# WasifurRahman/BERT_multimodal_transformer

Measured on AMD Instinct MI355X. Metric: train samples/sec MAG-BERT MOSI seq_len=50, higher is better.
Workload: dtype bf16; 1 GPU; MAG-BERT bert-base-uncased, MOSI dims (V=47, A=74), batch 48/GPU, seq_len 50, full optimizer step (fwd+MSE+bwd+HF-AdamW+schedule+zero_grad; inputs resident in HBM), dropout on, random-init weights; global_batch=48, seq_len=50, parallelism=dp1, step_call=mb_bert_train_step, hipGraph replay

## Files before the change

### bert_multimodal_transformer_amd/_lib.py

```python
import ctypes as C
import os

_HERE = os.path.dirname(os.path.abspath(__file__))
LIB_PATH = os.path.join(os.environ.get("MB_LIB_DIR") or os.path.join(_HERE, "lib"), "libmagbert_hip.so")

DT_F32, DT_BF16 = 0, 1
GEMM_NT, GEMM_NN, GEMM_TN = 0, 1, 2
EPI_BIAS, EPI_BIAS_GELU, EPI_BIAS_DROP_RES, EPI_ADD_RES, EPI_DGELU, EPI_ACCUM_F32, EPI_BIAS_F32 = range(7)


class DropKey(C.Structure):
    _fields_ = [("k0", C.c_uint32), ("k1", C.c_uint32), ("thresh", C.c_uint32), ("scale", C.c_float)]


class BertEngineConfig(C.Structure):
    _fields_ = [("vocab_size", C.c_int), ("hidden_size", C.c_int), ("num_layers", C.c_int), ("num_heads", C.c_int),
                ("intermediate_size", C.c_int), ("max_position", C.c_int), ("type_vocab", C.c_int),
                ("num_labels", C.c_int), ("visual_dim", C.c_int), ("acoustic_dim", C.c_int), ("pad_token_id", C.c_int),
                ("layer_norm_eps", C.c_float), ("mag_layer_norm_eps", C.c_float), ("beta_shift", C.c_float),
                ("hidden_dropout", C.c_float), ("attn_dropout", C.c_float), ("mag_dropout", C.c_float),
                ("dtype", C.c_int), ("max_batch", C.c_int), ("max_seq", C.c_int)]


class XlnetEngineConfig(C.Structure):
# ... 45 lines not shown
    "mb_bert_sequence_output": (_vp, [_vp]),
    "mb_bert_pooled_output": (_vp, [_vp]),
    "mb_bert_hidden_state": (_vp, [_vp, _i]),
    "mb_bert_set_attention_output": (_i, [_vp, _vp]),
    "mb_debug_gemm_trace": (_i, [_vp, _i]),
    "mb_debug_attention_trace": (_i, [_vp, _i]),
    "mb_xlnet_attention_probs": (_vp, [_vp, _i, C.POINTER(_i)]),
    "mb_xlnet_set_head_mask": (_i, [_vp, _vp]),
    "mb_xlnet_set_perm_mask": (_i, [_vp, _vp]),
    "mb_xlnet_set_mems": (_i, [_vp, _vp, _i]),
    "mb_xlnet_query_stream_scratch_bytes": (_sz, [_vp, _i, _i, _i]),
    "mb_xlnet_query_stream_state_bytes": (_sz, [_vp, _i, _i]),
    "mb_xlnet_query_stream": (_i, [_vp, _vp, _i, _vp, _sz, _vp, _vp]),
    "mb_bert_mark_grads_zero": (_i, [_vp, _i]),
    "mb_xlnet_mark_grads_zero": (_i, [_vp, _i]),
    "mb_bert_materialize_grads": (_i, [_vp, _vp]),
    "mb_xlnet_materialize_grads": (_i, [_vp, _vp]),
    "mb_bert_grads_stale": (_i, [_vp]),
    "mb_xlnet_grads_stale": (_i, [_vp]),
    "mb_bert_set_head_mask": (_i, [_vp, _vp]),
    "mb_bert_set_inputs_embeds": (_i, [_vp, _vp]),
    "mb_bert_set_position_ids": (_i, [_vp, _vp]),
    "mb_bert_inputs_embeds_grad": (_vp, [_vp]),
    "mb_bert_backward_outputs": (_i, [_vp, _vp, _vp, _vp]),
    "mb_bert_stage_grad_ranges": (_i, [_vp, _i, C.POINTER(_sz), C.POINTER(_sz), _i]),
    "mb_bert_train_step": (_i, [_vp, _vp, _vp, _vp, _vp, _vp, _vp, _i, _i, _u64, _u64, _vp, _vp, _vp, _vp, _vp, _f, _f, _f, _f, _f,
                                _i, _i, _f, _f, _i, _vp]),
    "mb_bert_stage_forward": (_i, [_vp, _vp, _vp, _vp, _vp, _vp, _vp, _i, _i, _u64, _u64, _vp, _vp, _vp, _i, _vp]),
    "mb_bert_stage_backward": (_i, [_vp, _f, _i, _i, _vp]),
    "mb_bert_staged_input_ids": (_vp, [_vp]),
# ... 107 lines not shown
```

### bert_multimodal_transformer_amd/bert.py

```python
import ctypes as C
import os

import torch
import torch.nn as nn

from . import _lib
from .global_configs import ACOUSTIC_DIM, VISUAL_DIM


class BertConfig(object):

    def __init__(self, vocab_size=30522, hidden_size=768, num_hidden_layers=12, num_attention_heads=12,
                 intermediate_size=3072, hidden_act="gelu", hidden_dropout_prob=0.1, attention_probs_dropout_prob=0.1,
                 max_position_embeddings=512, type_vocab_size=2, initializer_range=0.02, layer_norm_eps=1e-12,
                 pad_token_id=0, num_labels=1, **kwargs):
        if hidden_act != "gelu":
            raise NotImplementedError("only erf-GELU (bert-base-uncased) is built")
        self.vocab_size = vocab_size
        self.hidden_size = hidden_size
        self.num_hidden_layers = num_hidden_layers
        self.num_attention_heads = num_attention_heads
        self.intermediate_size = intermediate_size
        self.hidden_act = hidden_act
        self.hidden_dropout_prob = hidden_dropout_prob
# ... 393 lines not shown
        self._set_optional(None, None, None)
        ptr, keep = self._inputs(input_ids, visual, acoustic, attention_mask, token_type_ids, labels, gather_in_step=True)
        if not hasattr(self, "_logit_bufs"):
            self._logit_bufs = {}
        logits = self._logit_bufs.get(B)
        if logits is None:
            logits = self._logit_bufs[B] = torch.empty(B, self.config.num_labels, dtype=torch.float32, device=self.device)
        self.step += 1
        self._keep = (keep, logits)
        self._lab_ptr = None
        self.training_last = True
        o = opt or {}
        if comm is not None and opt is None:
            raise ValueError("the data-parallel single-call step ends with the optimizer (micro-steps exchange nothing)")
        extra = () if comm is None else (comm.handle,)
        with _Core._Hop(self):
            _lib.check(self._fn("train_step" if comm is None else "train_step_dp")(
                self.handle, ptr[0], ptr[1], ptr[2], ptr[3], ptr[4], ptr[5], B, L,
                self.seed & (2 ** 64 - 1), self.step, _lib.ptr(logits), C.c_void_p(self.loss_buf.data_ptr()),
                C.c_void_p(self.loss_buf.data_ptr() + 4), _lib.ptr(o.get("m")), _lib.ptr(o.get("v")), o.get("lr", 0.0),
                o.get("beta1", 0.9), o.get("beta2", 0.999), o.get("eps", 1e-6), o.get("weight_decay", 0.0), int(o.get("t", 1)),
                1 if o.get("correct_bias", True) else 0, o.get("grad_scale", 1.0), float(loss_scale), int(mode), self.stream(), *extra))
        self._gz = opt is not None
        self._gz_version = self.grads._version
        return logits

    def stage_step(self, input_ids, visual, acoustic, attention_mask, token_type_ids, labels, loss_scale=1.0, mode=1):
        B, L = input_ids.shape
        self._ensure(B, L)
        if self.weights_dirty:
# ... 514 lines not shown
```

### bert_multimodal_transformer_amd/csrc/adamw.hip

```cpp
#include <cstdlib>
#include "kernels.h"
#include "adamw_dev.h"

namespace mb {

template <bool NT, int UNR, bool CHUNK>
__global__ void __launch_bounds__(256) adamw_var_kernel(float* __restrict__ p, float* __restrict__ g, float* __restrict__ m,
                                                        float* __restrict__ v, bf16* __restrict__ shadow, size_t n4, size_t n_decay,
                                                        size_t sh_begin, size_t sh_end, size_t keep_begin, size_t keep_end, AdamArgs a,
                                                        const AdamArgs* __restrict__ dyn, int zero_grad) {
    if (dyn) a = *dyn;
    const float omb1 = 1.0f - a.beta1, omb2 = 1.0f - a.beta2;
    const float decay = a.lr * a.weight_decay;
    size_t begin, end, stride;
    if constexpr (CHUNK) {
        const size_t per = ((n4 + gridDim.x - 1) / gridDim.x + 255) / 256 * 256;
        begin = (size_t)blockIdx.x * per + threadIdx.x; end = min(n4, (size_t)(blockIdx.x + 1) * per); stride = 256;
    } else {
        begin = (size_t)blockIdx.x * 256 + threadIdx.x; end = n4; stride = (size_t)gridDim.x * 256;
    }
    for (size_t i4 = begin; i4 < end; i4 += stride * UNR) {
        AdamQuad q[UNR];
#pragma unroll
        for (int u = 0; u < UNR; ++u)
// ... 84 lines not shown
        const size_t kb = keep_begin, ke = keep_end;
        const int use = (var == 0 && ke > kb) ? 3 : var;
#define MB_AV(U, C) do { if (nt) hipLaunchKernelGGL((adamw_var_kernel<true, U, C>), dim3(grid), dim3(256), 0, st, p, g, m, v, (bf16*)shadow, n4, n_decay, sh_begin, sh_end, kb, ke, a, dyn, zero_grad); \
                         else hipLaunchKernelGGL((adamw_var_kernel<false, U, C>), dim3(grid), dim3(256), 0, st, p, g, m, v, (bf16*)shadow, n4, n_decay, sh_begin, sh_end, kb, ke, a, dyn, zero_grad); } while (0)
        if (use == 1) MB_AV(2, false); else if (use == 2) MB_AV(1, true); else if (use == 3) MB_AV(2, true); else if (use == 4) MB_AV(4, false); else if (use == 5) MB_AV(4, true); else
#undef MB_AV
        if (nt) hipLaunchKernelGGL(adamw_kernel<true>, dim3(grid), dim3(256), 0, st, p, g, m, v, (bf16*)shadow, n4, n_decay, sh_begin,
                                   sh_end, a, dyn, zero_grad);
        else hipLaunchKernelGGL(adamw_kernel<false>, dim3(grid), dim3(256), 0, st, p, g, m, v, (bf16*)shadow, n4, n_decay, sh_begin,
                                sh_end, a, dyn, zero_grad);
    }
    if (n % 4) hipLaunchKernelGGL(adamw_tail_kernel, dim3(1), dim3(64), 0, st, p, g, m, v, n4 * 4, n, n_decay, a, dyn, zero_grad);
    return (int)hipGetLastError();
}

}
```

### bert_multimodal_transformer_amd/csrc/adamw_dev.h

```cpp
#pragma once
#include "kernels.h"

namespace mb {

struct AdamQuad { f32x4 p, g, m, v; };
template <bool NT> __device__ __forceinline__ AdamQuad adam_load(const float* p, const float* g, const float* m, const float* v, size_t i) {
    AdamQuad q;
    if constexpr (NT) {
        q.p = __builtin_nontemporal_load((const f32x4*)(p + i)); q.g = __builtin_nontemporal_load((const f32x4*)(g + i));
        q.m = __builtin_nontemporal_load((const f32x4*)(m + i)); q.v = __builtin_nontemporal_load((const f32x4*)(v + i));
    } else {
        q.p = *(const f32x4*)(p + i); q.g = *(const f32x4*)(g + i); q.m = *(const f32x4*)(m + i); q.v = *(const f32x4*)(v + i);
    }
    return q;
}
template <bool NT> __device__ __forceinline__ void adam_update_store(AdamQuad q, float* p, float* g, float* m, float* v, bf16* shadow, size_t i,
                                                                     const AdamArgs& a, float omb1, float omb2, float decay, size_t n_decay,
                                                                     size_t sh_begin, size_t sh_end, size_t keep_begin, size_t keep_end, int zero_grad) {
#pragma clang fp contract(off)
    q.g *= a.grad_scale;
    q.m = a.beta1 * q.m + omb1 * q.g;
    q.v = a.beta2 * q.v + omb2 * q.g * q.g;
#pragma unroll
    for (int r = 0; r < 4; ++r) q.p[r] -= a.step_size * (q.m[r] / (sqrtf(q.v[r]) + a.eps));
    if (i < n_decay && decay > 0.f) q.p -= decay * q.p;
    const bool zg = zero_grad && !(i >= keep_begin && i < keep_end);
    if constexpr (NT) {
// ... 49 lines not shown
```

### bert_multimodal_transformer_amd/csrc/engine.hip

```cpp
#include "engine_common.h"
#include "comm.h"

struct LayerOff { size_t wqkv, wo, w1, w2, bqkv, bo, ln1w, ln1b, b1, b2, ln2w, ln2b; };
struct LayerWs { size_t qkv, ctx, s1, st1, y1, u, g, s2, st2, stats; };

struct mb_bert_engine : StepMixin {
    mb_bert_config c;
    std::vector<TensorInfo> tensors;
    std::vector<LayerOff> lo;
    size_t word, pos, type, emb_lnw, emb_lnb, wp, bp, wc, bc;
    size_t mag_whv, mag_wha, mag_wv, mag_wa, mag_bhv, mag_bha, mag_bv, mag_ba, mag_lnw, mag_lnb;
    size_t n_params, n_decay, sh_begin, sh_end;
    MagWs mw;
    size_t ws_mag, ws_emb, ws_emb_st, ws_head_z, ws_head_pooled, ws_logits;
    std::vector<size_t> ws_x;
    std::vector<LayerWs> lw;
    size_t ws_ds[2], ws_dzd[2], ws_ds2[2], ws_dzd2[2], ws_du[2], ws_dqkv[2];
    size_t ws_dxa, ws_dxb, ws_dctx, ws_dsum, ws_dz, ws_lnp_a, ws_lnp_b;
    size_t lnp_stride = 0;
    int lnp_nblk = 0;
    size_t ws_ids, ws_seg, ws_mask, ws_labels;
    size_t ws_bytes;
    float* P = nullptr; float* G = nullptr; char* SH = nullptr; char* ws = nullptr;
    const int64_t* ids = nullptr; const int64_t* seg = nullptr; const int64_t* mask = nullptr;
    int B = 0, L = 0, training = 0;
    int padT = -1;
    hipStream_t side = nullptr;
    std::vector<hipEvent_t> evs;
    int overlap_wgrad = 0;
    int opt_chunk = 0;
    int prefetch = 1;
    int pf_qkv = 0;
    hipStream_t opt_side = nullptr;
    std::vector<hipEvent_t> opt_ev;
    int adam_in_wgrad = 0;
    float* fuse_m = nullptr; float* fuse_v = nullptr;
    int adam_ride = 1, ride_blocks = 0;
    float* ride_m = nullptr; float* ride_v = nullptr;
    size_t ride_cursor = 0;
    long ride_params = 0;
    int ride_dgrad = 2, ride_dgrad_blocks = 0;
    int ride_attn = 1, ride_attn_blocks = 0;
    long ride_attn_params = 0;
    long ride_dgrad_params = 0, ride_dgelu_params = 0;
    int group_wgrad = 256;
    bool grouped = false;
    bool deferred = false;
    float* attn_out = nullptr;
    const float* head_mask = nullptr;
    const float* emb_in = nullptr;
    const int64_t* pos_ids = nullptr;
    bool ran_forward = false;

    bool ws_zeroed = false;
// ... 100 lines not shown
    e->ws_dxa = w.take(T * H * es); e->ws_dxb = w.take(T * H * es);
    for (int k = 0; k < 2; ++k) {
        e->ws_ds[k] = w.take(T * H * es); e->ws_dzd[k] = w.take(T * H * es); e->ws_ds2[k] = w.take(T * H * es);
        e->ws_dzd2[k] = w.take(T * H * es); e->ws_du[k] = w.take(T * I * es); e->ws_dqkv[k] = w.take(T * 3 * H * es);
    }
    e->ws_dctx = w.take(T * H * es); e->ws_dsum = w.take(T * H * 4); e->ws_dz = w.take((size_t)c.max_batch * H * es);
    e->lnp_stride = ln_partials_floats((int)T, (int)H);
    {
        const size_t emb = (size_t)c.max_seq * ((c.max_batch + 7) / 8) * 3 * H;
        if (emb > e->lnp_stride) e->lnp_stride = emb;
    }
    e->ws_lnp_a = w.take(e->lnp_stride * 4 * (c.num_layers + 2)); e->ws_lnp_b = w.take(e->lnp_stride * 4 * (c.num_layers + 2));
    e->carve_step(w, T, (int)V, (int)A, c.max_batch, c.num_labels, SITE_LAYER0 + 4 * c.num_layers);
    e->idcnt_off = w.take((size_t)c.vocab_size * 4);
    { const char* uv = getenv("MB_EMBED_UNIQUE"); e->idcnt_enable = !(uv && atoi(uv) == 0); }
    if (e->deterministic) {
        e->det_begin = e->wp; e->det_end = e->n_params;
        e->ws_det = w.take((e->det_end - e->det_begin) * sizeof(long long));
    }
    e->ws_bytes = w.off;
}

static int ensure_side(mb_bert_engine* e) {
    if (e->side || !e->overlap_wgrad) return MB_OK;
    int least = 0, greatest = 0;
    CK((int)hipDeviceGetStreamPriorityRange(&least, &greatest));
    const char* pv = getenv("MB_SIDE_PRIORITY");
    const int prio = (pv && atoi(pv) != 0) ? least : 0;
    CK((int)hipStreamCreateWithPriority(&e->side, hipStreamNonBlocking, prio));
    e->evs.assign((size_t)e->c.num_layers * 5, nullptr);
// ... 235 lines not shown
    if (ndim) *ndim = t.ndim;
    if (shape4) for (int k = 0; k < 4; ++k) shape4[k] = t.shape[k];
    if (decay) *decay = t.decay;
    return MB_OK;
}
size_t mb_bert_param_count(const mb_bert_engine* e) { return e->n_params; }
size_t mb_bert_decay_count(const mb_bert_engine* e) { return e->n_decay; }
void mb_bert_shadow_range(const mb_bert_engine* e, size_t* b, size_t* en) { *b = e->sh_begin; *en = e->sh_end; }
size_t mb_bert_workspace_bytes(const mb_bert_engine* e) { return e->ws_bytes; }

int mb_bert_bind(mb_bert_engine* e, float* params, float* grads, void* shadow, void* workspace, size_t ws_bytes) {
    if (!params || !workspace || ws_bytes < e->ws_bytes) return MB_ERR_ARG;
    if (e->c.dtype == DT_BF16 && !shadow) return MB_ERR_ARG;
    e->P = params; e->G = grads; e->SH = (char*)shadow; e->ws = (char*)workspace;
    e->grads_zero = false;
    e->ws_zeroed = false; e->padT = -1;
    e->drop_graphs();
    char* mws = e->ws + e->ws_mag;
    e->pkw = {e->P + e->mag_whv, e->P + e->mag_wha, e->P + e->mag_wv, e->P + e->mag_wa, mws + e->mw.We, mws + e->mw.Wv, mws + e->mw.Wa,
              MagDims{0, e->c.hidden_size, e->c.visual_dim, e->c.acoustic_dim, e->mw.Vp, e->mw.Ap}, e->c.dtype};
    return MB_OK;
}

int mb_bert_sync_weights(mb_bert_engine* e, void* stream) {
    hipStream_t st = (hipStream_t)stream;
    if (!e->P) return MB_ERR_ARG;
    if (e->c.dtype == DT_BF16)
        CK(convert(DT_BF16, e->P + e->sh_begin, e->SH + e->sh_begin * 2, e->sh_end - e->sh_begin, st));
    const mb_bert_config& c = e->c;
    MagDims d = {0, c.hidden_size, c.visual_dim, c.acoustic_dim, e->mw.Vp, e->mw.Ap};
// ... 60 lines not shown
    return MB_OK;
}

int mb_bert_forward(mb_bert_engine* e, const int64_t* input_ids, const float* visual, const float* acoustic,
                    const int64_t* attention_mask, const int64_t* token_type_ids, const float* labels, int B, int L,
                    int training, uint64_t seed, uint64_t step, float* logits, float* loss, float* loss_run, void* stream) {
    return bert_forward_range(e, input_ids, visual, acoustic, attention_mask, token_type_ids, labels, B, L, training, seed, step, logits,
                              loss, loss_run, stream, 0, e->c.num_layers, true, true);
}

int mb_bert_backward(mb_bert_engine* e, const float* dlogits, const float* labels, float loss_scale, int stage_begin,
                     int stage_end, void* stream) {
    hipStream_t st = (hipStream_t)stream;
    const mb_bert_config& c = e->c;
    if (!e->G || !e->ran_forward) return MB_ERR_ARG;
    const int dt = c.dtype, H = c.hidden_size, I = c.intermediate_size, B = e->B, L = e->L, T = B * L, nh = c.num_heads;
    const int NL = c.num_layers;
    const int Tk = (int)align_up((size_t)T, 64);
    auto take_ride = [&](int l, size_t budget, int blocks) -> AdamRide {
        AdamRide r = {};
        if (!e->ride_m || !e->ride_v || l + 1 >= e->c.num_layers || blocks < 8 || e->ride_cursor <= e->lo[l + 1].wqkv) return r;
        size_t take = std::min(e->ride_cursor - e->lo[l + 1].wqkv, budget) / 1024 * 1024;
        const size_t re = e->ride_cursor, rb = re - take;
        const bool sh_ok = e->c.dtype != DT_BF16 || (e->sh_begin <= rb && re <= e->sh_end);
        if (take == 0 || rb % 4 || !sh_ok) return r;
        const bool keep = e->keep_in_step() && e->stale_begin <= rb && re <= e->stale_end;
        r = AdamRide{e->P + rb, e->G + rb, e->ride_m + rb, e->ride_v + rb, e->c.dtype == DT_BF16 ? (bf16*)(e->SH + rb * 2) : nullptr,
                     take / 4, e->adam_state(e->ws), blocks / 8 * 8, keep ? 0 : 1};
        e->ride_cursor = rb;
        return r;
// ... 231 lines not shown
    const bool fuse = e->adam_in_wgrad && m && v && nseg == 1 && e->ow_pass && e->grouped && !e->deferred && e->group_wgrad == 128 && NL > 0 &&
                      e->lo[0].wqkv == 0 && !e->prof;
    e->fuse_m = fuse ? m : nullptr; e->fuse_v = fuse ? v : nullptr;
    const bool ride = e->adam_ride && !fuse && m && v && nseg == 1 && e->grouped && !e->deferred && NL > 1 && e->lo[0].wqkv == 0 && !e->prof &&
                      (e->group_wgrad == 128 || e->group_wgrad == 256);
    e->ride_m = ride ? m : nullptr; e->ride_v = ride ? v : nullptr;
    e->ride_cursor = e->wp;
    const int rb = mb_bert_backward(e, nullptr, lab, loss_scale, sb, se, st);
    e->fuse_m = e->fuse_v = nullptr;
    e->ride_m = e->ride_v = nullptr;
    CK(rb);
    if (m && v && seg == nseg - 1) {
        const AdamArgs none = {};
        const size_t nd = e->n_decay, n = e->n_params;
        CK(e->prof_mark(2 * NL, st));
        if (ride) CK(adamw_decay_range(e, m, v, 0, e->ride_cursor, st));
        CK(adamw_decay_range(e, m, v, (nseg == 1 && !fuse && !ride) ? 0 : e->wp, nd, st));
        CK(adamw_step(e->P + nd, e->G + nd, m + nd, v + nd, nullptr, n - nd, 0, 0, 0, none, 1, st, e->adam_state(ws) + 1));
        CK(e->prof_mark(2 * NL + 1, st));
    }
    return MB_OK;
}

static int between_segments(mb_bert_engine* e, int seg, int nseg, float* m, float* v, hipStream_t st) {
    if (nseg == 1 || !m || !v) return MB_OK;
    const int NL = e->c.num_layers, C = NL / (nseg - 1);
    if (seg + 1 < nseg) {
        const int l_lo = NL - (seg + 1) * C, l_hi = NL - seg * C;
        CK((int)hipEventRecord(e->opt_ev[seg], st));
        CK((int)hipStreamWaitEvent(e->opt_side, e->opt_ev[seg], 0));
// ... 234 lines not shown
    return e->prof_span_us(2 * e->c.num_layers, 1, us);
}

const void* mb_bert_hidden_state(const mb_bert_engine* e, int i) {
    if (!e || !e->ws || i < 0 || i > e->c.num_layers) return nullptr;
    return e->ws + e->ws_x[i];
}
int mb_bert_set_attention_output(mb_bert_engine* e, float* probs) {
    if (!e) return MB_ERR_ARG;
    e->attn_out = probs;
    return MB_OK;
}
int mb_bert_mark_grads_zero(mb_bert_engine* e, int known_zero) {
    if (!e) return MB_ERR_ARG;
    e->grads_zero = known_zero != 0;
    if (known_zero) e->grads_stale = false;
    return MB_OK;
}
int mb_bert_materialize_grads(mb_bert_engine* e, void* stream) {
    if (!e) return MB_ERR_ARG;
    return e->materialize_grads(e->G, (hipStream_t)stream);
}
int mb_bert_grads_stale(const mb_bert_engine* e) { return e && e->grads_stale ? 1 : 0; }
int mb_bert_set_head_mask(mb_bert_engine* e, const float* head_mask) {
    if (!e) return MB_ERR_ARG;
    e->head_mask = head_mask;
    return MB_OK;
}
int mb_bert_set_inputs_embeds(mb_bert_engine* e, const float* inputs_embeds) {
    if (!e) return MB_ERR_ARG;
    e->emb_in = inputs_embeds;
    return MB_OK;
}
// ... 62 lines not shown
```

### bert_multimodal_transformer_amd/csrc/engine_common.h

```cpp
#pragma once
#include <string>
#include <vector>
#include <cstring>
#include <cstdio>
#include <cstdlib>
#include <cmath>
#include <algorithm>
#include "kernels.h"
#include "../../include/magbert_hip.h"

using namespace mb;

namespace {

struct TensorInfo {
    std::string name;
    size_t off, numel;
    int ndim;
    int64_t shape[4];
    int decay;
};

inline size_t align_up(size_t x, size_t a) { return (x + a - 1) / a * a; }

// ... 149 lines not shown
        exec.clear(); graph.clear();
    }
};

struct StageGraph { int B, L, stage, overwrite; const void *logits, *loss, *loss_run; float loss_scale; hipStream_t st; hipGraph_t graph; hipGraphExec_t exec; };

struct StepMixin {
    bool dyn = false;
    bool stage_mode = false;
    std::vector<StageGraph> stage_graphs;
    bool pk_enable = false, packed = false;
    bool pkw_enable = false, packed_w = false;
    PrologueArgs::MagPackW pkw = {};
    size_t pk_vis = 0, pk_aco = 0; int pk_Vp = 0, pk_Ap = 0, pk_dtype = 0;
    size_t idcnt_off = 0; bool idcnt_enable = false, counted = false;
    bool loss_cleared = false;
    bool capturing = false;
    int nsites = 0;
    size_t ws_state = 0, ws_in_ids = 0, ws_in_seg = 0, ws_in_mask = 0, ws_in_vis = 0, ws_in_aco = 0, ws_in_lab = 0;
    std::vector<StepGraph> graphs;
    size_t graph_launches = 0, graph_captures = 0;
    hipStream_t cap = nullptr;
    int capture_stream(hipStream_t* out) {
        if (!cap) CK((int)hipStreamCreateWithFlags(&cap, hipStreamNonBlocking));
        *out = cap;
        return MB_OK;
    }
    bool grads_zero = false, ow_pass = false, in_step = false;
    int ow_enable = 1;
    int deterministic = 0;
// ... 11 lines not shown
            if (cus <= 0) cus = 256;
        }
        return cus;
    }
    bool grads_stale = false, ow_covers = false;
    size_t stale_begin = 0, stale_end = 0;
    int keep_enable = 1;
    bool keep_in_step() const { return keep_enable && ow_enable && ow_covers && stale_end > stale_begin; }
    int materialize_grads(float* G, hipStream_t st) {
        if (grads_stale && G) CK(zero_fill(G + stale_begin, (stale_end - stale_begin) * sizeof(float), st));
        grads_stale = false;
        return MB_OK;
    }
    int begin_backward_pass(float* G, hipStream_t st) {
        if (in_step) return MB_OK;
        ow_pass = grads_zero && ow_enable;
        grads_zero = false;
        if (!(ow_pass && ow_covers)) CK(materialize_grads(G, st));
        grads_stale = false;
        return MB_OK;
    }

    bool prof = false;
    std::vector<hipEvent_t> pev;
    int prof_layers = 0;
    int set_profiling(int on, int layers) {
        if (on && pev.empty()) {
            prof_layers = layers;
            pev.assign((size_t)2 * layers + 2, nullptr);
            for (auto& ev : pev) CK((int)hipEventCreate(&ev));
// ... 23 lines not shown
        ws_in_vis = w.take(Tpad * (size_t)V * 4); ws_in_aco = w.take(Tpad * (size_t)A * 4);
        ws_in_lab = w.take((size_t)max_batch * num_labels * 4);
    }
    void drop_graphs() {
        if (cap) { hipStreamDestroy(cap); cap = nullptr; }
        for (auto& g : graphs) g.destroy();
        graphs.clear();
        for (auto& g : stage_graphs) { hipGraphExecDestroy(g.exec); hipGraphDestroy(g.graph); }
        stage_graphs.clear();
    }
    template <class Enq>
    int run_stage_graph(int B, int L, int stage, int overwrite, const void* logits, const void* loss, const void* loss_run, float loss_scale,
                        int mode, hipStream_t st, Enq enqueue) {
        struct Scope { StepMixin* m; ~Scope() { m->dyn = false; m->capturing = false; m->in_step = false; m->stage_mode = false; } } scope{this};
        dyn = true; in_step = true; stage_mode = true;
        if (mode == 2) return enqueue(st);
        StageGraph* g = nullptr;
        for (auto& x : stage_graphs)
            if (x.B == B && x.L == L && x.stage == stage && x.overwrite == overwrite && x.logits == logits && x.loss == loss && x.loss_run == loss_run &&
                x.loss_scale == loss_scale && x.st == st) { g = &x; break; }
        if (!g) {
            if (stage_graphs.size() >= 256) {
                hipGraphExecDestroy(stage_graphs.front().exec); hipGraphDestroy(stage_graphs.front().graph);
                stage_graphs.erase(stage_graphs.begin());
            }
            StageGraph ng = {B, L, stage, overwrite, logits, loss, loss_run, loss_scale, st, nullptr, nullptr};
            hipStream_t cs = nullptr;
            CK(capture_stream(&cs));
            CK((int)hipStreamBeginCapture(cs, hipStreamCaptureModeRelaxed));
            capturing = true;
// ... 49 lines not shown
inline int train_step_impl(E* e, char* ws, int V, int A, int num_labels, const void* ids, const void* vis, const void* aco, const void* mask,
                           const void* seg, const void* labels, int B, int L, uint64_t seed, uint64_t step, float* logits, float* loss,
                           float* loss_run, float* m, float* v, float lr, float beta1, float beta2, float eps, float weight_decay,
                           int opt_step, int correct_bias, float grad_scale, float loss_scale, int mode, bool force_launches,
                           hipStream_t st, Enqueue enqueue_inner, int nseg = 1, Between between = Between(), int variant = 0,
                           const void* tag = nullptr, int (*verify)(const void* tag, int nseg, int sg, hipGraph_t gr) = nullptr) {
    const int ow = (e->grads_zero && e->ow_enable) ? 1 : 0;
    if (!(ow && e->ow_covers)) CK(e->materialize_grads(e->G, st));
    const bool stale_before = e->grads_stale;
    struct Flags {
        E* e; bool ok, with_opt, stale_before;
        ~Flags() {
            e->in_step = false; e->loss_cleared = false; e->packed = false; e->packed_w = false; e->counted = false;
            e->grads_zero = ok && with_opt;
            e->grads_stale = ok ? (with_opt && e->keep_in_step()) : stale_before;
        }
    } flags{e, false, m != nullptr, stale_before};
    e->in_step = true; e->ow_pass = ow != 0;
    auto enqueue = [&](int sg, float* lg, float* ls, float* lr_, float* m_, float* v_, float sc, hipStream_t s) {
        return enqueue_inner(sg, lg, ls, lr_, m_, v_, sc, s);
    };
    PrologueArgs pa = {};
    e->fill_copies(pa, ws, ids, vis, aco, mask, seg, labels, B, L, V, A, num_labels, e->pk_enable);
    e->packed = e->pk_enable;
    if (e->pkw_enable && e->pkw.W_hv) pa.magw = e->pkw;
    e->packed_w = pa.magw.W_hv != nullptr;
    pa.seed = seed; pa.step = step; pa.keys = e->key_state(ws); pa.nsites = e->nsites;
    pa.zero_dw = (uint32_t*)loss; e->loss_cleared = loss != nullptr;
    if (e->idcnt_enable && ids) { pa.ids = (const int64_t*)ids; pa.n_ids = B * L; pa.id_count = (int*)(ws + e->idcnt_off); }
    e->counted = pa.id_count != nullptr;
    if (m) {
        double ss = lr;
        if (correct_bias) ss = (double)lr * sqrt(1.0 - pow((double)beta2, (double)opt_step)) / (1.0 - pow((double)beta1, (double)opt_step));
        AdamArgs a;
        a.lr = lr; a.beta1 = beta1; a.beta2 = beta2; a.eps = eps; a.weight_decay = weight_decay; a.step_size = (float)ss;
        a.grad_scale = grad_scale;
        pa.adam[0] = a;
        a.weight_decay = 0.f;
        pa.adam[1] = a;
        pa.adam_dst = e->adam_state(ws);
    }
    CK(step_prologue(pa, st));
    if (mode == 2 || force_launches) {
        e->dyn = true;
        int r = MB_OK;
// ... 168 lines not shown
```

### bert_multimodal_transformer_amd/csrc/kernels.h

```cpp
#pragma once
#include <cstdio>
#include <cstdlib>
#include "common.h"

namespace mb {

enum {
    MB_OK = 0,
    MB_ERR_SHAPE = 1001,
    MB_ERR_MODE = 1002,
    MB_ERR_DTYPE = 1003,
    MB_ERR_ARG = 1004,
    MB_ERR_COMM = 1005,
};

inline void ck_trace(const char* expr, const char* file, int line, int code) {
    static int on = -1;
    if (on < 0) { const char* v = getenv("MB_CK_TRACE"); on = (v && atoi(v)) ? 1 : 0; }
    if (on) fprintf(stderr, "[magbert] %s:%d: %s -> %d\n", file, line, expr, code);
}

enum { GEMM_NT = 0,
       GEMM_NN = 1,
       GEMM_TN = 2 };
// ... 150 lines not shown
int last_token_backward(int dtype, const void* dxs, void* dx, int B, int L, int H, DropKey drop, hipStream_t st);
int xlnet_broadcast_row(int dtype, const float* row, void* out, int rows, int H, hipStream_t st);
int xlnet_map_query(int dtype, const float* tm, const void* qg, const void* qkv_h, void* qkv_g, int B, int M, int L, int H, hipStream_t st);
int xlnet_unmap_vec(int dtype, const float* tm, const void* vec, void* vecg, int B, int M, int L, int H, hipStream_t st);

int head_forward(const float* z, const float* Wc, const float* bc, const float* labels, float* pooled,
                 float* logits, float* loss, float* loss_run, int B, int H, int nl, DropKey drop, hipStream_t st);
int head_backward(int dtype, const float* dlogits, const float* logits, const float* labels, float loss_scale,
                  const float* pooled, const float* Wc, void* dz, float* dWc, float* dbc,
                  int B, int H, int nl, DropKey drop, hipStream_t st, GradAcc acc = {}, float* dbp = nullptr,
                  void* zero_p = nullptr, size_t zero_bytes = 0);

int adamw_step(float* p, float* g, float* m, float* v, void* shadow, size_t n, size_t n_decay,
               size_t sh_begin, size_t sh_end, AdamArgs a, int zero_grad, hipStream_t st, const AdamArgs* dyn = nullptr,
               size_t keep_begin = 0, size_t keep_end = 0);

#define MB_PROLOGUE_MAX_COPIES 8
struct PrologueArgs {
    const uint32_t* src[MB_PROLOGUE_MAX_COPIES]; uint32_t* dst[MB_PROLOGUE_MAX_COPIES]; uint32_t dwords[MB_PROLOGUE_MAX_COPIES];
    int ncopies;
    uint64_t seed, step;
    uint32_t* keys; int nsites;
    AdamArgs adam[2]; AdamArgs* adam_dst;
    uint32_t* zero_dw;
    struct PackJob { const float* src; void* dst; int rows, cols, pitch, dtype; } pack[2];
    int npack;
    const int64_t* ids; int n_ids; int* id_count;
    struct MagPackW { const float* W_hv; const float* W_ha; const float* W_v; const float* W_a; void* We; void* Wv; void* Wa; MagDims d; int dtype; } magw;
    int copy_blocks;
};
int step_prologue(const PrologueArgs& a, hipStream_t st);
#define MB_ZERO_MAX 8
struct ZeroRanges {
    uint32_t* p[MB_ZERO_MAX]; size_t ndw[MB_ZERO_MAX]; int n;
    void add(void* ptr, size_t bytes) { if (bytes && n < MB_ZERO_MAX) { p[n] = (uint32_t*)ptr; ndw[n] = bytes / 4; ++n; } }
    bool full() const { return n >= MB_ZERO_MAX; }
};
int zero_fill(void* p, size_t bytes, hipStream_t st);
int zero_fill_ranges(const ZeroRanges& z, hipStream_t st);

}
```

### bert_multimodal_transformer_amd/csrc/rowops.hip

```cpp
#include <algorithm>
#include "kernels.h"
#include "mag_pack.h"

namespace mb {

template <int CH>
struct RowStat {
    static __device__ __forceinline__ void compute(const f32x4 (&v)[CH], float eps, float& mu, float& rs) {
        constexpr float invH = 1.0f / (CH * 256);
        float s = 0.f;
#pragma unroll
        for (int c = 0; c < CH; ++c) s += (v[c][0] + v[c][1]) + (v[c][2] + v[c][3]);
        mu = wave_sum(s) * invH;
        float q = 0.f;
#pragma unroll
        for (int c = 0; c < CH; ++c) {
#pragma unroll
            for (int r = 0; r < 4; ++r) { const float d = v[c][r] - mu; q += d * d; }
        }
        rs = 1.0f / sqrtf(wave_sum(q) * invH + eps);
    }
};

template <class T, int CH>
// ... 696 lines not shown
        else mag_pack_w_range<float>(w.W_hv, w.W_ha, w.W_v, w.W_a, (float*)w.We, (float*)w.Wv, (float*)w.Wa, w.d, first, stride);
        return;
    }
    const size_t tid = (size_t)blockIdx.x * 256 + threadIdx.x, nth = (size_t)a.copy_blocks * 256;
    if (blockIdx.x == 0) {
        for (int s = threadIdx.x; s < a.nsites; s += 256) {
            const uint64_t h = splitmix64_dev(splitmix64_dev(a.seed) ^ splitmix64_dev(a.step * 0x100000001B3ull + (uint64_t)s));
            a.keys[2 * s] = (uint32_t)h;
            a.keys[2 * s + 1] = (uint32_t)(h >> 32);
        }
        if (a.adam_dst && threadIdx.x < 2) a.adam_dst[threadIdx.x] = a.adam[threadIdx.x];
    }
    if (tid == 0 && a.zero_dw) *a.zero_dw = 0u;
    if (a.id_count != nullptr)
        for (size_t i = tid; i < (size_t)a.n_ids; i += nth) atomicAdd(a.id_count + a.ids[i], 1);
    for (int k = 0; k < a.npack; ++k) {
        const PrologueArgs::PackJob& j = a.pack[k];
        const size_t n = (size_t)j.rows * j.cols;
        if ((((uintptr_t)j.src) & 15) == 0) {
            for (size_t i = tid; i < (n + 3) / 4; i += nth) {
                const size_t e0 = i * 4;
                f32x4 v = {0.f, 0.f, 0.f, 0.f};
                if (e0 + 4 <= n) v = __builtin_nontemporal_load((const f32x4*)j.src + i);
                else for (int r = 0; r < 4; ++r) if (e0 + r < n) v[r] = j.src[e0 + r];
                size_t row = e0 / j.cols;
                int c = (int)(e0 - row * j.cols);
#pragma unroll
                for (int r = 0; r < 4; ++r) {
                    if (e0 + r < n) {
                        const size_t d = row * j.pitch + c;
// ... 33 lines not shown
        }
        return;
    }
#pragma unroll 1
    for (int c = 0; c < a.ncopies; ++c) {
        const uint32_t* __restrict__ src = a.src[c];
        uint32_t* __restrict__ dst = a.dst[c];
        const size_t n = a.dwords[c];
        for (size_t i = tid; i < n; i += nth) dst[i] = src[i];
    }
}

int step_prologue(const PrologueArgs& a, hipStream_t st) {
    if (a.ncopies < 0 || a.ncopies > MB_PROLOGUE_MAX_COPIES || a.nsites < 0 || (a.nsites > 0 && !a.keys)) return MB_ERR_ARG;
    if (a.npack < 0 || a.npack > 2) return MB_ERR_ARG;
    size_t most = 0;
    for (int k = 0; k < a.npack; ++k) {
        if (!a.pack[k].src || !a.pack[k].dst || a.pack[k].cols < 1 || a.pack[k].pitch < a.pack[k].cols) return MB_ERR_ARG;
        most = std::max(most, (size_t)a.pack[k].rows * a.pack[k].cols);
    }
    for (int c = 0; c < a.ncopies; ++c) {
        if (a.dwords[c] && (!a.src[c] || !a.dst[c])) return MB_ERR_ARG;
        if (a.dwords[c] > most) most = a.dwords[c];
    }
    unsigned grid = (unsigned)((most / 4 + 255) / 256);
    if (grid < 1) grid = 1;
    if (grid > 512) grid = 512;
    PrologueArgs b = a;
    b.copy_blocks = (int)grid;
    if (a.magw.W_hv != nullptr) {
// ... 28 lines not shown
```

### include/magbert_hip.h

```cpp
#ifndef MAGBERT_HIP_H
#define MAGBERT_HIP_H
#include <stddef.h>
#include <stdint.h>

#ifdef __cplusplus
extern "C" {
#endif

#define MB_DT_F32 0
#define MB_DT_BF16 1

typedef struct { uint32_t k0, k1, thresh; float scale; } mb_dropkey;

const char* mb_error_string(int code);
int mb_version(void);
void mb_make_dropkey(uint64_t seed, uint64_t step, uint32_t site, float p, mb_dropkey* out);


int mb_gemm(int dtype, int layout, int epilogue, int M, int N, int K, const void* A, int lda, const void* B, int ldb,
            void* C, int ldc, void* C2, float* Cf, const float* bias, const void* R, int ldr, float alpha,
            const mb_dropkey* drop, int splits, int tile, void* stream);

int mb_debug_gemm_trace(unsigned long long* host_out, int max_blocks);
int mb_debug_attention_trace(unsigned long long* host_out, int max_blocks);
// ... 74 lines not shown
                    void* stream);
int mb_bert_backward(mb_bert_engine* e, const float* dlogits, const float* labels, float loss_scale, int stage_begin,
                     int stage_end, void* stream);
const void* mb_bert_sequence_output(const mb_bert_engine* e);
const float* mb_bert_pooled_output(const mb_bert_engine* e);
const void* mb_bert_hidden_state(const mb_bert_engine* e, int i);
int mb_bert_set_attention_output(mb_bert_engine* e, float* probs);
int mb_bert_set_head_mask(mb_bert_engine* e, const float* head_mask);
int mb_bert_set_inputs_embeds(mb_bert_engine* e, const float* inputs_embeds);
int mb_bert_set_position_ids(mb_bert_engine* e, const int64_t* position_ids);
const float* mb_bert_inputs_embeds_grad(const mb_bert_engine* e);
int mb_bert_backward_outputs(mb_bert_engine* e, const void* d_sequence_output, const void* d_pooler_preact, void* stream);
int mb_bert_stage_grad_ranges(const mb_bert_engine* e, int stage, size_t* offs, size_t* lens, int cap);

int mb_bert_mark_grads_zero(mb_bert_engine* e, int known_zero);
int mb_bert_materialize_grads(mb_bert_engine* e, void* stream);
int mb_bert_grads_stale(const mb_bert_engine* e);

int mb_bert_train_step(mb_bert_engine* e, const int64_t* input_ids, const float* visual, const float* acoustic,
                       const int64_t* attention_mask, const int64_t* token_type_ids, const float* labels, int B, int L,
                       uint64_t seed, uint64_t step, float* logits, float* loss, float* loss_run, float* m, float* v, float lr,
                       float beta1, float beta2, float eps, float weight_decay, int opt_step, int correct_bias, float grad_scale,
                       float loss_scale, int mode, void* stream);
int mb_bert_stage_forward(mb_bert_engine* e, const int64_t* input_ids, const float* visual, const float* acoustic,
                          const int64_t* attention_mask, const int64_t* token_type_ids, const float* labels, int B, int L,
                          uint64_t seed, uint64_t step, float* logits, float* loss, float* loss_run, int mode, void* stream);
int mb_bert_stage_backward(mb_bert_engine* e, float loss_scale, int stage, int mode, void* stream);
const int64_t* mb_bert_staged_input_ids(const mb_bert_engine* e);
int mb_bert_load_batch(mb_bert_engine* e, const int64_t* input_ids, const float* visual, const float* acoustic,
                       const int64_t* attention_mask, const int64_t* token_type_ids, const float* labels, int B, int L,
// ... 107 lines not shown
```

Baseline: 14700 samples/s.

## Fuse AdamW ranges into one sweep and skip grad reads for untouched word rows

Replaces the several AdamW launches with a single sweep kernel that walks all parameter ranges (decay, no-decay, ride). It also stamps the word-embedding rows seen in the batch during the step prologue, and the sweep skips loading gradients for rows whose gradients are known to be zero. The aim is to save launch overhead and HBM reads of the large word-embedding gradient (vocab × hidden). The cost is extra stamp-tracking state and the correctness risk of trusting zero-gradient stamps, which a Python hook resets when the grads tensor changes.

```diff
diff --git a/bert_multimodal_transformer_amd/_lib.py b/bert_multimodal_transformer_amd/_lib.py
--- a/bert_multimodal_transformer_amd/_lib.py
+++ b/bert_multimodal_transformer_amd/_lib.py
@@ -83,6 +83,8 @@
     "mb_xlnet_query_stream": (_i, [_vp, _vp, _i, _vp, _sz, _vp, _vp]),
     "mb_bert_mark_grads_zero": (_i, [_vp, _i]),
     "mb_xlnet_mark_grads_zero": (_i, [_vp, _i]),
+    "mb_bert_distrust_word_stamps": (_i, [_vp]),
+    "mb_bert_word_skip_updates": (_sz, [_vp]),
     "mb_bert_materialize_grads": (_i, [_vp, _vp]),
     "mb_xlnet_materialize_grads": (_i, [_vp, _vp]),
     "mb_bert_grads_stale": (_i, [_vp]),
diff --git a/bert_multimodal_transformer_amd/bert.py b/bert_multimodal_transformer_amd/bert.py
--- a/bert_multimodal_transformer_amd/bert.py
+++ b/bert_multimodal_transformer_amd/bert.py
@@ -431,6 +431,8 @@
         if comm is not None and opt is None:
             raise ValueError("the data-parallel single-call step ends with the optimizer (micro-steps exchange nothing)")
         extra = () if comm is None else (comm.handle,)
+        if self.kind == "bert" and self.grads._version != getattr(self, "_gz_version", -1):
+            _lib.check(self.lib.mb_bert_distrust_word_stamps(self.handle))
         with _Core._Hop(self):
             _lib.check(self._fn("train_step" if comm is None else "train_step_dp")(
                 self.handle, ptr[0], ptr[1], ptr[2], ptr[3], ptr[4], ptr[5], B, L,
diff --git a/bert_multimodal_transformer_amd/csrc/adamw.hip b/bert_multimodal_transformer_amd/csrc/adamw.hip
--- a/bert_multimodal_transformer_amd/csrc/adamw.hip
+++ b/bert_multimodal_transformer_amd/csrc/adamw.hip
@@ -122,4 +122,80 @@
     return (int)hipGetLastError();
 }
 
-}
+template <bool NT>
+__global__ void __launch_bounds__(256) adamw_sweep_kernel(float* __restrict__ p, float* __restrict__ g, float* __restrict__ m,
+                                                          float* __restrict__ v, bf16* __restrict__ shadow, AdamRanges R, size_t n_decay,
+                                                          size_t sh_begin, size_t sh_end, size_t keep_begin, size_t keep_end,
+                                                          const AdamArgs* __restrict__ dyn, WordSkip ws) {
+    constexpr int UNR = 2;
+    size_t total4 = 0;
+    for (int k = 0; k < MB_SWEEP_MAX; ++k) if (k < R.count) total4 += R.n[k] / 4;
+    const size_t per = ((total4 + gridDim.x - 1) / gridDim.x + 255) / 256 * 256;
+    const size_t vb = (size_t)blockIdx.x * per, ve = min(total4, vb + per);
+    const bool skip_on = ws.stamp != nullptr && ws.state[1] != 0u;
+    const uint32_t stamp_no = skip_on ? ws.state[0] : 0u;
+    size_t off = 0;
+#pragma unroll 1
+    for (int k = 0; k < R.count; ++k) {
+        const size_t n4 = R.n[k] / 4;
+        const size_t lo = max(vb, off), hi = min(ve, off + n4);
+        off += n4;
+        if (lo >= hi) continue;
+        const AdamArgs a = dyn[R.slot[k]];
+        const float omb1 = 1.0f - a.beta1, omb2 = 1.0f - a.beta2;
+        const float decay = a.lr * a.weight_decay;
+        const size_t base4 = R.begin[k] / 4 + n4 - off;
+        const size_t begin = base4 + lo + threadIdx.x, end = base4 + hi;
+        for (size_t i4 = begin; i4 < end; i4 += 256 * UNR) {
+            AdamQuad q[UNR];
+            bool live[UNR];
+#pragma unroll
+            for (int u = 0; u < UNR; ++u) {
+                const size_t i = (i4 + (size_t)u * 256) * 4;
+                live[u] = true;
+                if (i4 + (size_t)u * 256 < end) {
+                    if (skip_on && i >= ws.begin && i < ws.end) live[u] = ws.stamp[(uint32_t)(i - ws.begin) / ws.row_len] == stamp_no;
+                    q[u] = adam_load<NT>(p, g, m, v, i, live[u]);
+                }
+            }
+#pragma unroll
+            for (int u = 0; u < UNR; ++u)
+                if (i4 + (size_t)u * 256 < end)
+                    adam_update_store<NT>(q[u], p, g, m, v, shadow, (i4 + (size_t)u * 256) * 4, a, omb1, omb2, decay, n_decay, sh_begin, sh_end,
+                                          keep_begin, keep_end, live[u] ? 1 : 0);
+        }
+    }
+}
+
+int adamw_sweep(float* p, float* g, float* m, float* v, void* shadow, const AdamRanges& r, size_t n_decay, size_t sh_begin, size_t sh_end,
+                size_t keep_begin, size_t keep_end, const AdamArgs* dyn, const WordSkip& skip, hipStream_t st) {
+    if (r.count < 0 || r.count > MB_SWEEP_MAX || !dyn) return MB_ERR_ARG;
+    size_t n = 0;
+    for (int k = 0; k < r.count; ++k) {
+        if ((r.begin[k] | r.n[k]) % 4 || r.slot[k] < 0 || r.slot[k] > 1) return MB_ERR_SHAPE;
+        n += r.n[k];
+    }
+    if (n == 0) return MB_OK;
+    if ((n_decay % 4) || (sh_begin % 4) || (sh_end % 4) || (keep_begin % 4) || (keep_end % 4)) return MB_ERR_SHAPE;
+    if (((uintptr_t)p | (uintptr_t)g | (uintptr_t)m | (uintptr_t)v) & 15) return MB_ERR_SHAPE;
+    if (skip.stamp && (!skip.state || skip.row_len == 0 || (skip.begin | skip.end | skip.row_len) % 4 || skip.end < skip.begin ||
+                       skip.end - skip.begin > 0xffffffffull)) return MB_ERR_SHAPE;
+    {
+        static int log = -1;
+        if (log < 0) { const char* e = getenv("MB_GEMM_LOG"); log = e ? atoi(e) : 0; }
+        if (log) fprintf(stderr, "[magbert adamw] n=%zu\n", n);
+    }
+    const size_t n4 = n / 4;
+    unsigned grid = (unsigned)((n4 + 255) / 256);
+    if (grid > 256 * 16) grid = 256 * 16;
+    static int nt = -1, vgrid = 0;
+    if (nt < 0) { const char* e = getenv("MB_ADAMW_NT"); nt = e ? atoi(e) : 1; const char* g2 = getenv("MB_ADAMW_GRID"); vgrid = g2 ? atoi(g2) : 0; }
+    if (vgrid > 0 && (unsigned)vgrid < grid) grid = (unsigned)vgrid;
+    if (nt) hipLaunchKernelGGL(adamw_sweep_kernel<true>, dim3(grid), dim3(256), 0, st, p, g, m, v, (bf16*)shadow, r, n_decay, sh_begin, sh_end,
+                               keep_begin, keep_end, dyn, skip);
+    else hipLaunchKernelGGL(adamw_sweep_kernel<false>, dim3(grid), dim3(256), 0, st, p, g, m, v, (bf16*)shadow, r, n_decay, sh_begin, sh_end,
+                            keep_begin, keep_end, dyn, skip);
+    return (int)hipGetLastError();
+}
+
+}
diff --git a/bert_multimodal_transformer_amd/csrc/adamw_dev.h b/bert_multimodal_transformer_amd/csrc/adamw_dev.h
--- a/bert_multimodal_transformer_amd/csrc/adamw_dev.h
+++ b/bert_multimodal_transformer_amd/csrc/adamw_dev.h
@@ -11,6 +11,20 @@
         q.m = __builtin_nontemporal_load((const f32x4*)(m + i)); q.v = __builtin_nontemporal_load((const f32x4*)(v + i));
     } else {
         q.p = *(const f32x4*)(p + i); q.g = *(const f32x4*)(g + i); q.m = *(const f32x4*)(m + i); q.v = *(const f32x4*)(v + i);
+    }
+    return q;
+}
+template <bool NT> __device__ __forceinline__ AdamQuad adam_load(const float* p, const float* g, const float* m, const float* v, size_t i, bool live) {
+    AdamQuad q;
+    q.g = f32x4{0.f, 0.f, 0.f, 0.f};
+    if constexpr (NT) {
+        q.p = __builtin_nontemporal_load((const f32x4*)(p + i));
+        if (live) q.g = __builtin_nontemporal_load((const f32x4*)(g + i));
+        q.m = __builtin_nontemporal_load((const f32x4*)(m + i)); q.v = __builtin_nontemporal_load((const f32x4*)(v + i));
+    } else {
+        q.p = *(const f32x4*)(p + i);
+        if (live) q.g = *(const f32x4*)(g + i);
+        q.m = *(const f32x4*)(m + i); q.v = *(const f32x4*)(v + i);
     }
     return q;
 }
diff --git a/bert_multimodal_transformer_amd/csrc/engine.hip b/bert_multimodal_transformer_amd/csrc/engine.hip
--- a/bert_multimodal_transformer_amd/csrc/engine.hip
+++ b/bert_multimodal_transformer_amd/csrc/engine.hip
@@ -38,6 +38,7 @@
     int adam_ride = 1, ride_blocks = 0;
     float* ride_m = nullptr; float* ride_v = nullptr;
     size_t ride_cursor = 0;
+    bool one_sweep = true;
     long ride_params = 0;
     int ride_dgrad = 2, ride_dgrad_blocks = 0;
     int ride_attn = 1, ride_attn_blocks = 0;
@@ -168,6 +169,10 @@
     e->carve_step(w, T, (int)V, (int)A, c.max_batch, c.num_labels, SITE_LAYER0 + 4 * c.num_layers);
     e->idcnt_off = w.take((size_t)c.vocab_size * 4);
     { const char* uv = getenv("MB_EMBED_UNIQUE"); e->idcnt_enable = !(uv && atoi(uv) == 0); }
+    e->stamp_rows = (size_t)c.vocab_size;
+    e->stamp_off = w.take(((size_t)c.vocab_size + 2) * 4);
+    { const char* sv = getenv("MB_ADAMW_SKIP_ZERO_ROWS"); e->stamp_enable = !(sv && atoi(sv) == 0); }
+    { const char* ov = getenv("MB_ADAMW_ONE_SWEEP"); e->one_sweep = !(ov && atoi(ov) == 0); }
     if (e->deterministic) {
         e->det_begin = e->wp; e->det_end = e->n_params;
         e->ws_det = w.take((e->det_end - e->det_begin) * sizeof(long long));
@@ -433,6 +438,7 @@
     if (e->c.dtype == DT_BF16 && !shadow) return MB_ERR_ARG;
     e->P = params; e->G = grads; e->SH = (char*)shadow; e->ws = (char*)workspace;
     e->grads_zero = false;
+    e->stamp_live = e->word_zero = false; e->sweep_no = 1;
     e->ws_zeroed = false; e->padT = -1;
     e->drop_graphs();
     char* mws = e->ws + e->ws_mag;
@@ -523,6 +529,7 @@
     hipStream_t st = (hipStream_t)stream;
     const mb_bert_config& c = e->c;
     if (!e->G || !e->ran_forward) return MB_ERR_ARG;
+    if (!e->in_step) e->stamp_live = e->word_zero = false;
     const int dt = c.dtype, H = c.hidden_size, I = c.intermediate_size, B = e->B, L = e->L, T = B * L, nh = c.num_heads;
     const int NL = c.num_layers;
     const int Tk = (int)align_up((size_t)T, 64);
@@ -784,6 +791,29 @@
         const AdamArgs none = {};
         const size_t nd = e->n_decay, n = e->n_params;
         CK(e->prof_mark(2 * NL, st));
+        const bool skip = e->stamp_off != 0 && e->stamp_enable && e->idcnt_enable;
+        if (nseg == 1 && (e->one_sweep || skip)) {
+            AdamRanges all = {};
+            auto add = [&](size_t b, size_t en, int slot) {
+                if (en > b) { all.begin[all.count] = b; all.n[all.count] = en - b; all.slot[all.count] = slot; ++all.count; }
+            };
+            if (ride) add(0, e->ride_cursor, 0);
+            add((!fuse && !ride) ? 0 : e->wp, nd, 0);
+            add(nd, n, 1);
+            const bool keep = e->keep_in_step();
+            WordSkip ws_ = {};
+            if (skip) ws_ = WordSkip{e->stamp_table(ws), e->stamp_state(ws), e->word, e->word + (size_t)e->c.vocab_size * e->c.hidden_size,
+                                      (uint32_t)e->c.hidden_size};
+            void* sh = e->c.dtype == DT_BF16 ? (void*)e->SH : nullptr;
+            for (int k = 0; k < (e->one_sweep ? 1 : all.count); ++k) {
+                AdamRanges one = all;
+                if (!e->one_sweep) { one = AdamRanges{}; one.begin[0] = all.begin[k]; one.n[0] = all.n[k]; one.slot[0] = all.slot[k]; one.count = 1; }
+                CK(adamw_sweep(e->P, e->G, m, v, sh, one, nd, e->sh_begin, e->sh_end, keep ? e->stale_begin : 0, keep ? e->stale_end : 0,
+                               e->adam_state(ws), ws_, st));
+            }
+            CK(e->prof_mark(2 * NL + 1, st));
+            return MB_OK;
+        }
         if (ride) CK(adamw_decay_range(e, m, v, 0, e->ride_cursor, st));
         CK(adamw_decay_range(e, m, v, (nseg == 1 && !fuse && !ride) ? 0 : e->wp, nd, st));
         CK(adamw_step(e->P + nd, e->G + nd, m + nd, v + nd, nullptr, n - nd, 0, 0, 0, none, 1, st, e->adam_state(ws) + 1));
@@ -1048,9 +1078,16 @@
 int mb_bert_mark_grads_zero(mb_bert_engine* e, int known_zero) {
     if (!e) return MB_ERR_ARG;
     e->grads_zero = known_zero != 0;
+    if (!known_zero) e->stamp_live = e->word_zero = false;
     if (known_zero) e->grads_stale = false;
     return MB_OK;
 }
+int mb_bert_distrust_word_stamps(mb_bert_engine* e) {
+    if (!e) return MB_ERR_ARG;
+    e->stamp_live = e->word_zero = false;
+    return MB_OK;
+}
+size_t mb_bert_word_skip_updates(const mb_bert_engine* e) { return e ? e->skip_updates : 0; }
 int mb_bert_materialize_grads(mb_bert_engine* e, void* stream) {
     if (!e) return MB_ERR_ARG;
     return e->materialize_grads(e->G, (hipStream_t)stream);
diff --git a/bert_multimodal_transformer_amd/csrc/engine_common.h b/bert_multimodal_transformer_amd/csrc/engine_common.h
--- a/bert_multimodal_transformer_amd/csrc/engine_common.h
+++ b/bert_multimodal_transformer_amd/csrc/engine_common.h
@@ -187,6 +187,11 @@
     PrologueArgs::MagPackW pkw = {};
     size_t pk_vis = 0, pk_aco = 0; int pk_Vp = 0, pk_Ap = 0, pk_dtype = 0;
     size_t idcnt_off = 0; bool idcnt_enable = false, counted = false;
+    size_t stamp_off = 0, stamp_rows = 0; bool stamp_enable = false, stamp_live = false, word_zero = false;
+    uint32_t sweep_no = 1;
+    size_t skip_updates = 0;
+    uint32_t* stamp_table(char* ws) const { return (uint32_t*)(ws + stamp_off); }
+    uint32_t* stamp_state(char* ws) const { return stamp_table(ws) + stamp_rows; }
     bool loss_cleared = false;
     bool capturing = false;
     int nsites = 0;
@@ -228,6 +233,7 @@
     }
     int begin_backward_pass(float* G, hipStream_t st) {
         if (in_step) return MB_OK;
+        stamp_live = word_zero = false;
         ow_pass = grads_zero && ow_enable;
         grads_zero = false;
         if (!(ow_pass && ow_covers)) CK(materialize_grads(G, st));
@@ -281,6 +287,7 @@
                         int mode, hipStream_t st, Enq enqueue) {
         struct Scope { StepMixin* m; ~Scope() { m->dyn = false; m->capturing = false; m->in_step = false; m->stage_mode = false; } } scope{this};
         dyn = true; in_step = true; stage_mode = true;
+        stamp_live = word_zero = false;
         if (mode == 2) return enqueue(st);
         StageGraph* g = nullptr;
         for (auto& x : stage_graphs)
@@ -360,8 +367,16 @@
             e->in_step = false; e->loss_cleared = false; e->packed = false; e->packed_w = false; e->counted = false;
             e->grads_zero = ok && with_opt;
             e->grads_stale = ok ? (with_opt && e->keep_in_step()) : stale_before;
+            if (ok && with_opt && e->stamp_live) ++e->skip_updates;
+            if (!ok || with_opt) e->stamp_live = false;
+            e->word_zero = ok && with_opt;
+            if (ok && with_opt && ++e->sweep_no == 0u) e->sweep_no = 1u;
         }
     } flags{e, false, m != nullptr, stale_before};
+    const bool stamping = e->stamp_off != 0 && e->stamp_enable && e->idcnt_enable && ids != nullptr;
+    if (!stamping) e->stamp_live = false;
+    else if (e->word_zero) e->stamp_live = true;
+    e->word_zero = false;
     e->in_step = true; e->ow_pass = ow != 0;
     auto enqueue = [&](int sg, float* lg, float* ls, float* lr_, float* m_, float* v_, float sc, hipStream_t s) {
         return enqueue_inner(sg, lg, ls, lr_, m_, v_, sc, s);
@@ -375,6 +390,7 @@
     pa.zero_dw = (uint32_t*)loss; e->loss_cleared = loss != nullptr;
     if (e->idcnt_enable && ids) { pa.ids = (const int64_t*)ids; pa.n_ids = B * L; pa.id_count = (int*)(ws + e->idcnt_off); }
     e->counted = pa.id_count != nullptr;
+    if (stamping) { pa.stamp = e->stamp_table(ws); pa.stamp_state = e->stamp_state(ws); pa.stamp_no = e->sweep_no; pa.stamp_on = e->stamp_live ? 1u : 0u; }
     if (m) {
         double ss = lr;
         if (correct_bias) ss = (double)lr * sqrt(1.0 - pow((double)beta2, (double)opt_step)) / (1.0 - pow((double)beta1, (double)opt_step));
diff --git a/bert_multimodal_transformer_amd/csrc/kernels.h b/bert_multimodal_transformer_amd/csrc/kernels.h
--- a/bert_multimodal_transformer_amd/csrc/kernels.h
+++ b/bert_multimodal_transformer_amd/csrc/kernels.h
@@ -188,6 +188,11 @@
 int adamw_step(float* p, float* g, float* m, float* v, void* shadow, size_t n, size_t n_decay,
                size_t sh_begin, size_t sh_end, AdamArgs a, int zero_grad, hipStream_t st, const AdamArgs* dyn = nullptr,
                size_t keep_begin = 0, size_t keep_end = 0);
+#define MB_SWEEP_MAX 4
+struct AdamRanges { size_t begin[MB_SWEEP_MAX], n[MB_SWEEP_MAX]; int slot[MB_SWEEP_MAX]; int count; };
+struct WordSkip { const uint32_t* stamp; const uint32_t* state; size_t begin, end; uint32_t row_len; };
+int adamw_sweep(float* p, float* g, float* m, float* v, void* shadow, const AdamRanges& r, size_t n_decay, size_t sh_begin, size_t sh_end,
+                size_t keep_begin, size_t keep_end, const AdamArgs* dyn, const WordSkip& skip, hipStream_t st);
 
 #define MB_PROLOGUE_MAX_COPIES 8
 struct PrologueArgs {
@@ -200,6 +205,7 @@
     struct PackJob { const float* src; void* dst; int rows, cols, pitch, dtype; } pack[2];
     int npack;
     const int64_t* ids; int n_ids; int* id_count;
+    uint32_t* stamp; uint32_t* stamp_state; uint32_t stamp_no, stamp_on;
     struct MagPackW { const float* W_hv; const float* W_ha; const float* W_v; const float* W_a; void* We; void* Wv; void* Wa; MagDims d; int dtype; } magw;
     int copy_blocks;
 };
diff --git a/bert_multimodal_transformer_amd/csrc/rowops.hip b/bert_multimodal_transformer_amd/csrc/rowops.hip
--- a/bert_multimodal_transformer_amd/csrc/rowops.hip
+++ b/bert_multimodal_transformer_amd/csrc/rowops.hip
@@ -734,6 +734,10 @@
     if (tid == 0 && a.zero_dw) *a.zero_dw = 0u;
     if (a.id_count != nullptr)
         for (size_t i = tid; i < (size_t)a.n_ids; i += nth) atomicAdd(a.id_count + a.ids[i], 1);
+    if (a.stamp != nullptr) {
+        for (size_t i = tid; i < (size_t)a.n_ids; i += nth) a.stamp[a.ids[i]] = a.stamp_no;
+        if (tid < 2) a.stamp_state[tid] = tid == 0 ? a.stamp_no : a.stamp_on;
+    }
     for (int k = 0; k < a.npack; ++k) {
         const PrologueArgs::PackJob& j = a.pack[k];
         const size_t n = (size_t)j.rows * j.cols;
@@ -797,6 +801,7 @@
 int step_prologue(const PrologueArgs& a, hipStream_t st) {
     if (a.ncopies < 0 || a.ncopies > MB_PROLOGUE_MAX_COPIES || a.nsites < 0 || (a.nsites > 0 && !a.keys)) return MB_ERR_ARG;
     if (a.npack < 0 || a.npack > 2) return MB_ERR_ARG;
+    if (a.stamp && (!a.stamp_state || !a.ids)) return MB_ERR_ARG;
     size_t most = 0;
     for (int k = 0; k < a.npack; ++k) {
         if (!a.pack[k].src || !a.pack[k].dst || a.pack[k].cols < 1 || a.pack[k].pitch < a.pack[k].cols) return MB_ERR_ARG;
diff --git a/include/magbert_hip.h b/include/magbert_hip.h
--- a/include/magbert_hip.h
+++ b/include/magbert_hip.h
@@ -112,6 +112,8 @@
 int mb_bert_stage_grad_ranges(const mb_bert_engine* e, int stage, size_t* offs, size_t* lens, int cap);
 
 int mb_bert_mark_grads_zero(mb_bert_engine* e, int known_zero);
+int mb_bert_distrust_word_stamps(mb_bert_engine* e);
+size_t mb_bert_word_skip_updates(const mb_bert_engine* e);
 int mb_bert_materialize_grads(mb_bert_engine* e, void* stream);
 int mb_bert_grads_stale(const mb_bert_engine* e);
 
```

Result: faster. 14880 samples/s (median of 6 runs) (+1.2%).
